# ihmcrobotics/mecano

Hardware: AMD Instinct MI355X
Metric: robot-configs/sec (RNEA+ABA), 30-DoF humanoid batch=4096 (higher is better)
Workload: dtype f64; 1 GPU; 30-DoF humanoid (SixDoF pelvis + 24 revolute), RNEA and ABA of every configuration per step, fp64, AoS [B][n] state; entry_point=mh_rnea_aba_f64, batch_per_gpu=4096, global_batch=4096, nq=31, nv=30, bodies=25, parallelism=dp1 (batch sharded, no data-path collective), kernel_variant=topo:b5c1e26c784c54fa, model_seed=43, state_seed=2342

## Files before the change

mecano_amd/csrc/mh_spec.hip:

```cpp
#include "mh_spec_kernels.h"
#include "mh_zv_kernels.h"

#include <algorithm>
#include <atomic>
#include <cstdlib>
#include <type_traits>

#ifndef MH_SPEC_PART
#define MH_SPEC_PART 0
#endif
#ifndef MH_TOPO_N
#error "MH_TOPO_N / MH_TOPO_PARENTS / MH_TOPO_TYPES must be defined"
#endif

namespace
{
struct TP
{
   static constexpr int N = MH_TOPO_N;
   static constexpr int parent[N] = {MH_TOPO_PARENTS};
   static constexpr int type[N] = {MH_TOPO_TYPES};
};
constexpr int kParents[TP::N] = {MH_TOPO_PARENTS};
constexpr int kTypes[TP::N] = {MH_TOPO_TYPES};
// ... 143 lines not shown
      return launch_lds(&mh::spec_fused_split_kernel<TP, double, ID, IO>, A, 2 * groups,
                        (size_t)split_lds_bytes(2, IO ? F_IO_LDS : 0, A.m.nq, A.m.nv), attr_bytes, stream);
   }
   else
      return hipErrorNotSupported;
}
template <int ALGO, bool ID, bool IO>
hipError_t go_split(const mh::Args<double> &A, int groups, hipStream_t stream, bool occ3 = false)
{
   if constexpr (SPL::usable())
   {
      static LdsAttr attr_bytes, attr_occ3;
      if constexpr (ALGO == 0 && ID && !IO)
      {
         if (occ3)
            return launch_lds(&mh::spec_split_kernel_occ3<TP, double, ALGO, ID, IO>, A, groups,
                              (size_t)split_lds_bytes(ALGO, 0, A.m.nq, A.m.nv), attr_occ3, stream);
      }
      return launch_lds(&mh::spec_split_kernel<TP, double, ALGO, ID, IO>, A, groups,
                        (size_t)split_lds_bytes(ALGO, IO ? F_IO_LDS : 0, A.m.nq, A.m.nv), attr_bytes, stream);
   }
   else
      return hipErrorNotSupported;
}
template <bool ID, bool IO>
hipError_t go_split_algo(int algo, const mh::Args<double> &A, int groups, hipStream_t s, bool occ3)
{
   if (algo == 2)
      return go_fused_split<ID, IO>(A, groups, s);
   if (algo == 0)
      return go_split<0, ID, IO>(A, groups, s, occ3);
   if (algo == 1)
      return go_split<1, ID, IO>(A, groups, s);
   return hipErrorNotSupported;
}

extern "C" {
#if MH_SPEC_PART != 2
int mh_spec_split_usable(void) { return SPL::usable() ? 1 : 0; }
long mh_spec_split_lds_bytes(int algo, int flags, int nq, int nv) { return split_lds_bytes(algo, flags, nq, nv); }
int mh_spec_launch_split(int algo, int flags, const void *args, int groups, void *stream)
{
   const mh::Args<double> &A = *(const mh::Args<double> *)args;
   const bool id = flags & F_IDENT, io = flags & F_IO_LDS;
   hipStream_t s = (hipStream_t)stream;
   const bool occ3 = (flags & F_OCC3) != 0;
   if (flags & F_BODIES)
   {
#ifdef MH_SPEC_MINIMAL
      return (int)hipErrorNotSupported;
#else
      if constexpr (SPL::usable())
      {
         if (id && io && (algo == 0 || algo == 1))
         {
            static LdsAttr attr0, attr1;
            const size_t lds = (size_t)split_lds_bytes(algo, F_IO_LDS, A.m.nq, A.m.nv);
            if (algo == 0)
               return (int)launch_lds(&mh::spec_split_kernel<TP, double, 0, true, true, true>, A, groups, lds, attr0, s);
            return (int)launch_lds(&mh::spec_split_kernel<TP, double, 1, true, true, true>, A, groups, lds, attr1, s);
         }
      }
      return (int)hipErrorNotSupported;
#endif
   }
   if (id && io)
      return (int)go_split_algo<true, true>(algo, A, groups, s, occ3);
#ifdef MH_SPEC_MINIMAL
   return (int)hipErrorNotSupported;
#else
   if (id)
      return (int)go_split_algo<true, false>(algo, A, groups, s, occ3);
   if (io)
      return (int)go_split_algo<false, true>(algo, A, groups, s, occ3);
   return (int)go_split_algo<false, false>(algo, A, groups, s, occ3);
#endif
}
#endif
#if MH_SPEC_PART != 1
long mh_spec_zv_lds_bytes(int nq, int nv)
{
   if constexpr (!SPL::usable())
      return 0;
   const long inertia = (long)(SPL::n_limbs() * mh::ZV_XW + SPL::ZV_TRUNK_SLOTS + nq + 2 * nv) * 64 * (long)sizeof(double);
   return std::max(inertia, split_lds_bytes(0, F_IO_LDS, nq, nv) + (long)mh::zv_bias_extra_rows<TP>() * 64 * (long)sizeof(double));
}
int mh_spec_zv_usable(void) { return SPL::usable() ? 1 : 0; }
int mh_spec_zv_self_signal(void) { return MH_ZV_TWO_STAGE && MH_ZV_SELF_SIGNAL ? 1 : 0; }
#ifdef MH_ZV_PROBE
int mh_spec_zv_probe_read(void *dst, size_t bytes) { return (int)hipMemcpyFromSymbol(dst, HIP_SYMBOL(mh::zv_probe), bytes); }
int mh_spec_zv_probe_body_read(void *dst, size_t bytes) { return (int)hipMemcpyFromSymbol(dst, HIP_SYMBOL(mh::zv_probe_body), bytes); }
#endif
int mh_spec_launch_zv(int flags, const void *args, void *taup, int *sync_flags, int *error, int epoch, int jobs, int same_l2, unsigned wait_ticks, void *stream)
{
   if constexpr (SPL::usable())
   {
      const mh::Args<double> &A = *(const mh::Args<double> *)args;
      if (!(flags & F_IO_LDS) || (jobs != 2 && jobs != 3))
         return (int)hipErrorNotSupported;
      const size_t lds = (size_t)mh_spec_zv_lds_bytes(A.m.nq, A.m.nv);
      if (lds > 160 * 1024)
         return (int)hipErrorNotSupported;
      const long groups = (A.B + 63) / 64, padded = (groups + 7) / 8 * 8;
      const mh::ZvSync sy{sync_flags, error, epoch, jobs, same_l2 ? 1 : 0, wait_ticks};
      hipStream_t s = (hipStream_t)stream;
      if (A.q_next && (!(flags & F_IDENT) || jobs != 2 || !MH_ZV_TWO_STAGE))
         return (int)hipErrorNotSupported;
      if ((flags & F_IDENT) && A.q_next)
      {
         static LdsAttr attr_step;
         auto kern = &mh::spec_zv_kernel<TP, double, true, true>;
         if (const hipError_t e = ensure_lds_attr(reinterpret_cast<const void *>(kern), lds, attr_step); e != hipSuccess)
            return (int)e;
         hipLaunchKernelGGL(kern, dim3((unsigned)(padded * jobs)), dim3(256), lds, s, A.q, A.qd, A.in3b, A.B, jobs, A, (double *)taup, sy);
         return (int)hipGetLastError();
      }
      if (flags & F_IDENT)
      {
         static LdsAttr attr;
         auto kern = &mh::spec_zv_kernel<TP, double, true>;
         if (const hipError_t e = ensure_lds_attr(reinterpret_cast<const void *>(kern), lds, attr); e != hipSuccess)
            return (int)e;
         hipLaunchKernelGGL(kern, dim3((unsigned)(padded * jobs)), dim3(256), lds, s, A.q, A.qd, A.in3b, A.B, jobs, A, (double *)taup, sy);
         return (int)hipGetLastError();
      }
#ifdef MH_SPEC_MINIMAL
      return (int)hipErrorNotSupported;
#else
      static LdsAttr attr2;
      auto kern = &mh::spec_zv_kernel<TP, double, false>;
      if (const hipError_t e = ensure_lds_attr(reinterpret_cast<const void *>(kern), lds, attr2); e != hipSuccess)
         return (int)e;
      hipLaunchKernelGGL(kern, dim3((unsigned)(padded * jobs)), dim3(256), lds, s, A.q, A.qd, A.in3b, A.B, jobs, A, (double *)taup, sy);
      return (int)hipGetLastError();
#endif
   }
   else
      return (int)hipErrorNotSupported;
}
int mh_spec_zvb_usable(void)
{
   if constexpr (SPL::usable())
      return mh::ZvbPlan<TP>::lds_slots() * 64 * (long)sizeof(double) * 2 <= 160 * 1024 ? 1 : 0;
   else
      return 0;
}
int mh_spec_zvb_cs_rows(void) { return 2 * TR::n_revolute(); }
long mh_spec_zvb_lds_bytes(int which, int nq, int nv)
{
   if constexpr (SPL::usable())
      return (long)(which == 0 ? mh::ZvbPlan<TP>::bias_lds_slots(nq, nv) : mh::ZvbPlan<TP>::lds_slots()) * 64 * (long)sizeof(double);
   else
      return 0;
}
int mh_spec_launch_zvb(int flags, const void *args, void *taup, void *cs, long cs_stride, int groups, int which, void *stream)
{
   if constexpr (SPL::usable())
   {
      const mh::Args<double> &A = *(const mh::Args<double> *)args;
      if (!(flags & F_IO_LDS) || !mh_spec_zvb_usable() || cs_stride < (A.B + 63) / 64 * 64 || groups < 1)
         return (int)hipErrorNotSupported;
      const size_t lds0 = (size_t)mh_spec_zvb_lds_bytes(0, A.m.nq, A.m.nv), lds1 = (size_t)mh_spec_zvb_lds_bytes(1, A.m.nq, A.m.nv);
      if (lds0 > 160 * 1024)
         return (int)hipErrorNotSupported;
      hipStream_t s = (hipStream_t)stream;
      auto run = [&](auto ident) -> hipError_t {
         constexpr bool ID = decltype(ident)::value;
// ... 309 lines not shown
```

mecano_amd/csrc/mh_zv_kernels.h:

```cpp
#pragma once
#include "mh_spec_kernels.h"

namespace mh
{
template <class TP>
struct ZvStore
{
   static constexpr int REG_SLOTS = Split<TP>::zv_reg_slots();
   static constexpr int kind(int j) { return Split<TP>::is_trunk(j) ? ST_LDS_KIND : ST_REG_KIND; }
   static constexpr int index(int j) { return Split<TP>::is_trunk(j) ? Split<TP>::zv_trunk_slot(j) : Split<TP>::zv_reg_slot(j); }
   static constexpr bool shared(int j) { return !Split<TP>::is_trunk(j); }
};
template <class TP>
struct ZvbStore
{
   using S = Split<TP>;
   static constexpr bool root_in_regs(int j) { return S::staged() && j == S::root(); }
   static constexpr int REG_SLOTS = S::zv_reg_slots() + (S::staged() ? Tree<TP>::zv_slots_of(S::root() < 0 ? 0 : S::root(), true) : 0);
   static constexpr int trunk_slot(int j)
   {
      int s = 0;
      for (int i = 0; i < j; i++)
         s += S::is_trunk(i) && !root_in_regs(i) ? Tree<TP>::zv_slots_of(i, false) : 0;
      return s;
// ... 427 lines not shown
         else if constexpr (MODE == 2)
            c = x_get6<Split<TP>::sub_slot(C), CX::fold_xw, 6, CX, T>(cx);
         else
            c = ZvFold<TP, C, T, CX, MODE>::run(cx);
         if constexpr (K == 0)
            pA = c;
         else
            pA = pA + c;
         children<K + 1>(cx, pA);
      }
   }
   static MH_DEV SV<T> run(const CX &cx)
   {
      MH_BODY_FENCE();
      constexpr int TYPE = TP::type[J];
      constexpr bool HAS_PARENT = TP::parent[J] >= 0;
      constexpr bool LEAF = Tree<TP>::n_children(J) == 0;
      constexpr int DO = Tree<TP>::dof_ofs(J), CO = Tree<TP>::cfg_ofs(J);
      constexpr int RS = Tree<TP>::zv_result_slot(J, CX::SPolicy::shared(J));
      const V3<T> Z{T(0), T(0), T(0)};
      SV<T> pA{Z, Z};
      if constexpr (!LEAF)
         children<0>(cx, pA);
      MH_BODY_FENCE();
      ZV_STAMP_TAIL(J, 0);
      const T *cp = cx.C + J * MC_STRIDE;
      asm volatile("" : "+s"(cp));
      const CRef<T> c{cp};
      SV<T> up{Z, Z};
      if constexpr (TYPE == JT_REVOLUTE || TYPE == JT_PRISMATIC)
      {
         T tau;
         if constexpr (CX::csmode == 3)
            tau = zvf_tau_get1<TP, J, 0, CX, T>(cx);
         else
            tau = cx.in3(DO);
         JX<T> jx;
         jx.c = T(1), jx.s = T(0), jx.d = T(0);
         if constexpr (TYPE == JT_REVOLUTE)
            jx.c = cx.st.template get<J, 7>(), jx.s = cx.st.template get<J, 8>();
         else if constexpr (HAS_PARENT)
            jx.d = cx.q(CO);
         const V3<T> sa{cx.st.template get<J, 0>(), cx.st.template get<J, 1>(), cx.st.template get<J, 2>()};
         const V3<T> sl{cx.st.template get<J, 3>(), cx.st.template get<J, 4>(), cx.st.template get<J, 5>()};
         const T dinv = cx.st.template get<J, 6>();
         const T u = tau - (TYPE == JT_REVOLUTE ? pA.a.z : pA.l.z);
         cx.st.template put<J, RS>(u * dinv);
         if constexpr (HAS_PARENT)
         {
            const XF<T> Xb = load_xb_j<TP, J, T>(c);
            const SV<T> pa = pA + SV<T>{u * sa, u * sl};
            up = force_up(TYPE, jx, Xb, pa);
         }
      }
      else if constexpr (TYPE == JT_SIXDOF)
      {
         SV<T> tau;
         if constexpr (CX::csmode == 3)
            tau = SV<T>{V3<T>{zvf_tau_get1<TP, J, 0, CX, T>(cx), zvf_tau_get1<TP, J, 1, CX, T>(cx), zvf_tau_get1<TP, J, 2, CX, T>(cx)},
                        V3<T>{zvf_tau_get1<TP, J, 3, CX, T>(cx), zvf_tau_get1<TP, J, 4, CX, T>(cx), zvf_tau_get1<TP, J, 5, CX, T>(cx)}};
         else
            tau = spec_vec<TYPE, DO, 1, CX, T>(cx, true);
         const SV<T> x = spd6_solve(st_get_ldl<J, CX, T>(cx), tau - pA);
         cx.st.template put<J, RS + 0>(x.a.x), cx.st.template put<J, RS + 1>(x.a.y), cx.st.template put<J, RS + 2>(x.a.z);
         cx.st.template put<J, RS + 3>(x.l.x), cx.st.template put<J, RS + 4>(x.l.y), cx.st.template put<J, RS + 5>(x.l.z);
         if constexpr (HAS_PARENT)
         {
            const JX<T> jx = spec_joint<TYPE, CO, CX, T>(cx);
            up = force_up(TYPE, jx, load_xb_j<TP, J, T>(c), tau);
         }
      }
      else if constexpr (HAS_PARENT)
      {
         JX<T> jx;
         jx.c = T(1), jx.s = T(0), jx.d = T(0);
         up = force_up(TYPE, jx, load_xb_j<TP, J, T>(c), pA);
      }
      MH_BODY_FENCE();
      ZV_STAMP_TAIL(J, 1);
      return up;
   }
};

template <class TP, int J, typename T, class CX, int MODE = 0>
struct ZvOut
{
   template <int K>
   static MH_DEV void children(const CX &cx, const SV<T> &a)
   {
      if constexpr (K < Tree<TP>::n_children(J))
      {
         constexpr int C = Tree<TP>::child(J, K);
         if constexpr (MODE == 1 && !Split<TP>::is_trunk(C))
         {
            if (cx.wave == Split<TP>::owner(Split<TP>::limb_index(C)))
               ZvOut<TP, C, T, CX, 0>::run(cx, a);
         }
         else
            ZvOut<TP, C, T, CX, MODE>::run(cx, a);
         children<K + 1>(cx, a);
      }
   }
   static MH_DEV void run(const CX &cx, const SV<T> &ap)
   {
      MH_BODY_FENCE();
      constexpr int TYPE = TP::type[J];
      constexpr bool HAS_PARENT = TP::parent[J] >= 0;
      constexpr bool LEAF = Tree<TP>::n_children(J) == 0;
      constexpr int DO = Tree<TP>::dof_ofs(J), CO = Tree<TP>::cfg_ofs(J);
      constexpr int RS = Tree<TP>::zv_result_slot(J, CX::SPolicy::shared(J));
      ZV_STAMP_TAIL(J, 2);
      const T *cp = cx.C + J * MC_STRIDE;
      asm volatile("" : "+s"(cp));
      const CRef<T> c{cp};
      const V3<T> Z{T(0), T(0), T(0)};
      SV<T> a{Z, Z};
      if constexpr (HAS_PARENT)
      {
         JX<T> jx;
         jx.c = T(1), jx.s = T(0), jx.d = T(0);
         if constexpr (TYPE == JT_REVOLUTE)
            jx.c = cx.st.template get<J, 7>(), jx.s = cx.st.template get<J, 8>();
         else if constexpr (TYPE != JT_FIXED)
            jx = spec_joint<TYPE, CO, CX, T>(cx);
         a = motion_down(TYPE, jx, load_xb_j<TP, J, T>(c), ap);
      }
      if constexpr (TYPE == JT_REVOLUTE || TYPE == JT_PRISMATIC)
      {
         const V3<T> sa{cx.st.template get<J, 0>(), cx.st.template get<J, 1>(), cx.st.template get<J, 2>()};
         const V3<T> sl{cx.st.template get<J, 3>(), cx.st.template get<J, 4>(), cx.st.template get<J, 5>()};
         const T qdd = cx.st.template get<J, RS>() - (dot(sa, a.a) + dot(sl, a.l));
         if (MODE == 0 || cx.wave == 0)
            cx.out(DO, qdd);
         if constexpr (TYPE == JT_REVOLUTE)
            a.a.z += qdd;
         else
            a.l.z += qdd;
      }
      else if constexpr (TYPE == JT_SIXDOF)
      {
         const SV<T> x{V3<T>{cx.st.template get<J, RS + 0>(), cx.st.template get<J, RS + 1>(), cx.st.template get<J, RS + 2>()},
                       V3<T>{cx.st.template get<J, RS + 3>(), cx.st.template get<J, RS + 4>(), cx.st.template get<J, RS + 5>()}};
         if (MODE == 0 || cx.wave == 0)
            spec_write<TYPE, DO, CX, T>(cx, x - a);
         a = x;
      }
      MH_BODY_FENCE();
      ZV_STAMP_TAIL(J, 3);
      if constexpr (!LEAF)
         children<0>(cx, a);
   }
};

template <class TP, typename T, class CX, int MODE, int K = 0>
MH_DEV void zv_roots_in(const CX &cx)
{
   if constexpr (K < Tree<TP>::n_children(-1))
   {
      (void)ZvIn<TP, Tree<TP>::child(-1, K), T, CX, MODE>::run(cx);
      zv_roots_in<TP, T, CX, MODE, K + 1>(cx);
   }
}
template <class TP, typename T, class CX, int K = 0>
MH_DEV void zv_roots_fold(const CX &cx)
{
   if constexpr (K < Tree<TP>::n_children(-1))
   {
      (void)ZvFold<TP, Tree<TP>::child(-1, K), T, CX, 1>::run(cx);
      zv_roots_fold<TP, T, CX, K + 1>(cx);
   }
}
template <class TP, typename T, class CX, int K = 0>
MH_DEV void zv_roots_out(const CX &cx)
{
   if constexpr (K < Tree<TP>::n_children(-1))
   {
      const V3<T> Z{T(0), T(0), T(0)};
      ZvOut<TP, Tree<TP>::child(-1, K), T, CX, 1>::run(cx, SV<T>{Z, Z});
      zv_roots_out<TP, T, CX, K + 1>(cx);
   }
}
template <class TP, int W, int K, int LATE, typename T, class CX>
MH_DEV void zv_limbs_in_of(const CX &cx)
{
   using S = Split<TP>;
   if constexpr (K < S::n_limbs())
   {
      if constexpr (S::owner(K) == W && (LATE < 0 || (S::is_late(K) ? 1 : 0) == LATE))
      {
         if constexpr (CX::csmode != 3 && !(CX::csmode == 0 && MH_ZV_PRE_WAVE))
            zv_pre<TP, S::limb_root(K), T, CX>(cx);
         x_put_ia<K, CX, T>(cx, ZvIn<TP, S::limb_root(K), T, CX, (LATE >= 0 && S::cut_limb(W) == K ? 3 : 0)>::run(cx));
      }
      zv_limbs_in_of<TP, W, K + 1, LATE, T, CX>(cx);
   }
}
template <class TP, int W, int I, typename T, class CX>
MH_DEV void zv_subtrunks_of(const CX &cx)
{
   using S = Split<TP>;
   if constexpr (I < S::n_sub())
   {
      constexpr int ST = S::sub_top(I);
      if constexpr (S::sub_owner(ST) == W)
         x_put_ia<S::sub_slot(ST), CX, T>(cx, ZvIn<TP, ST, T, CX, 1>::run(cx));
      zv_subtrunks_of<TP, W, I + 1, T, CX>(cx);
   }
}
template <class TP, int W, int J, typename T, class CX>
MH_DEV void zvf_park_late_tau(const CX &cx)
{
   using SP = typename CX::SPolicy;
   if constexpr (J < TP::N)
   {
      if constexpr (SP::late_body(J) && Split<TP>::owner(Split<TP>::limb_index_of_body(J)) == W)
      {
         constexpr int TS = SP::tau_slot(J), L0 = SP::late_tau_slot(J);
         cx.st.lbase[L0 * 64] = cx.st.template get<J, TS>();
         if constexpr (Tree<TP>::ndof(J) == 6)
         {
            cx.st.lbase[(L0 + 1) * 64] = cx.st.template get<J, TS + 1>(), cx.st.lbase[(L0 + 2) * 64] = cx.st.template get<J, TS + 2>();
            cx.st.lbase[(L0 + 3) * 64] = cx.st.template get<J, TS + 3>(), cx.st.lbase[(L0 + 4) * 64] = cx.st.template get<J, TS + 4>();
            cx.st.lbase[(L0 + 5) * 64] = cx.st.template get<J, TS + 5>();
         }
      }
      zvf_park_late_tau<TP, W, J + 1, T, CX>(cx);
   }
}
template <class TP, int W, typename T, class CX>
MH_DEV void zv_limbs_in(const CX &cx)
{
   using S = Split<TP>;
// ... 57 lines not shown
struct zv_relay
{
   static constexpr bool value = false;
};
template <class CX>
struct zv_relay<CX, std::enable_if_t<CX::relay>>
{
   static constexpr bool value = true;
};
template <class TP, bool RELAY = false>
struct ZvWalk
{
   using S = Split<TP>;
   static constexpr bool below(int j, int top)
   {
      for (int a = j; a >= 0; a = TP::parent[a])
         if (a == top)
            return true;
      return false;
   }
   static constexpr bool owns_late(int W)
   {
      for (int k = 0; k < S::n_limbs(); k++)
         if (S::owner(k) == W && S::is_late(k))
            return true;
      return false;
   }
   static constexpr int poster(int k)
   {
      if (!RELAY || !S::staged() || S::is_late(k) || !owns_late(S::owner(k)) || TP::parent[S::limb_root(k)] == S::root())
         return -1;
      for (int w = 0; w < 4; w++)
         if (!owns_late(w) && ZvWalk<TP, false>::needs(w, TP::parent[S::limb_root(k)]))
            return w;
      return -1;
   }
   static constexpr bool relayed(int k) { return poster(k) >= 0; }
   static constexpr bool needs(int W, int J)
   {
      for (int k = 0; k < S::n_limbs(); k++)
         if (S::owner(k) == W && below(S::limb_root(k), J) && !relayed(k))
            return true;
      return false;
   }
   static constexpr int writer(int J)
   {
      for (int w = 0; w < 4; w++)
         if (needs(w, J))
            return w;
      return 0;
   }
};
constexpr int ZV_RELAY_A = 12, ZV_RELAY_FLAG = 18;
template <class TP, int J, int W, int K, typename T, class CX>
MH_DEV void zv_relay_post(const CX &cx, const SV<T> &a)
{
   using S = Split<TP>;
   if constexpr (K < S::n_limbs())
   {
      if constexpr (TP::parent[S::limb_root(K)] == J && ZvWalk<TP, true>::poster(K) == W)
      {
         x_put6<K, ZV_XW, ZV_RELAY_A, CX, T>(cx, a);
         asm volatile("s_waitcnt lgkmcnt(0)" ::: "memory");
         __hip_atomic_store(cx.xbase + (K * ZV_XW + ZV_RELAY_FLAG) * 64, T(1), __ATOMIC_RELAXED, __HIP_MEMORY_SCOPE_WORKGROUP);
      }
      zv_relay_post<TP, J, W, K + 1, T, CX>(cx, a);
   }
}
template <class TP, int W, int K, typename T, class CX>
MH_DEV void zv_relay_clear(const CX &cx)
{
   using S = Split<TP>;
   if constexpr (K < S::n_limbs())
   {
      if constexpr (S::owner(K) == W && ZvWalk<TP, true>::relayed(K))
         x_put<K, ZV_XW, ZV_RELAY_FLAG, CX, T>(cx, T(0));
      zv_relay_clear<TP, W, K + 1, T, CX>(cx);
   }
}
template <class TP, int J, int W, typename T, class CX>
struct ZvOutW
{
   using WK = ZvWalk<TP, zv_relay<CX>::value>;
   template <int K>
   static MH_DEV void children(const CX &cx, const SV<T> &a)
   {
      if constexpr (K < Tree<TP>::n_children(J))
      {
         constexpr int C = Tree<TP>::child(J, K);
         if constexpr (!Split<TP>::is_trunk(C))
         {
            if constexpr (Split<TP>::owner(Split<TP>::limb_index(C)) == W && !WK::relayed(Split<TP>::limb_index(C)))
               ZvOut<TP, C, T, CX, 0>::run(cx, a);
         }
         else if constexpr (WK::needs(W, C))
            ZvOutW<TP, C, W, T, CX>::run(cx, a);
         children<K + 1>(cx, a);
      }
   }
   static MH_DEV void run(const CX &cx, const SV<T> &ap)
   {
      MH_BODY_FENCE();
      constexpr int TYPE = TP::type[J];
      constexpr bool HAS_PARENT = TP::parent[J] >= 0;
      constexpr int DO = Tree<TP>::dof_ofs(J), CO = Tree<TP>::cfg_ofs(J);
      constexpr int RS = Tree<TP>::zv_result_slot(J, CX::SPolicy::shared(J));
      constexpr bool WRITES = WK::writer(J) == W;
      if constexpr (WRITES)
         ZV_STAMP_TAIL(J, 2);
      const T *cp = cx.C + J * MC_STRIDE;
      asm volatile("" : "+s"(cp));
      const CRef<T> c{cp};
      const V3<T> Z{T(0), T(0), T(0)};
      SV<T> a{Z, Z};
      if constexpr (HAS_PARENT)
      {
         JX<T> jx;
         jx.c = T(1), jx.s = T(0), jx.d = T(0);
         if constexpr (TYPE == JT_REVOLUTE)
            jx.c = cx.st.template get<J, 7>(), jx.s = cx.st.template get<J, 8>();
         else if constexpr (TYPE != JT_FIXED)
            jx = spec_joint<TYPE, CO, CX, T>(cx);
         a = motion_down(TYPE, jx, load_xb_j<TP, J, T>(c), ap);
      }
      if constexpr (TYPE == JT_REVOLUTE || TYPE == JT_PRISMATIC)
      {
         const V3<T> sa{cx.st.template get<J, 0>(), cx.st.template get<J, 1>(), cx.st.template get<J, 2>()};
         const V3<T> sl{cx.st.template get<J, 3>(), cx.st.template get<J, 4>(), cx.st.template get<J, 5>()};
         const T qdd = cx.st.template get<J, RS>() - (dot(sa, a.a) + dot(sl, a.l));
         if constexpr (WRITES)
            cx.out(DO, qdd);
         if constexpr (TYPE == JT_REVOLUTE)
            a.a.z += qdd;
         else
            a.l.z += qdd;
      }
      else if constexpr (TYPE == JT_SIXDOF)
      {
         const SV<T> x{V3<T>{cx.st.template get<J, RS + 0>(), cx.st.template get<J, RS + 1>(), cx.st.template get<J, RS + 2>()},
                       V3<T>{cx.st.template get<J, RS + 3>(), cx.st.template get<J, RS + 4>(), cx.st.template get<J, RS + 5>()}};
         if constexpr (WRITES)
            spec_write<TYPE, DO, CX, T>(cx, x - a);
         a = x;
      }
      MH_BODY_FENCE();
      if constexpr (WRITES)
         ZV_STAMP_TAIL(J, 3);
      if constexpr (zv_relay<CX>::value)
         zv_relay_post<TP, J, W, 0, T, CX>(cx, a);
      children<0>(cx, a);
   }
};
template <class TP, int W, typename T, class CX, int K = 0>
MH_DEV void zv_roots_out_wave(const CX &cx)
{
   if constexpr (K < Tree<TP>::n_children(-1))
   {
      const V3<T> Z{T(0), T(0), T(0)};
      constexpr int R = Tree<TP>::child(-1, K);
      using WK = ZvWalk<TP, zv_relay<CX>::value>;
      if constexpr (WK::needs(W, R) || WK::writer(R) == W)
         ZvOutW<TP, R, W, T, CX>::run(cx, SV<T>{Z, Z});
      zv_roots_out_wave<TP, W, T, CX, K + 1>(cx);
   }
}
template <class TP, int W, int K, typename T, class CX>
MH_DEV void zv_relay_out(const CX &cx)
{
   using S = Split<TP>;
   if constexpr (K < S::n_limbs())
   {
      if constexpr (S::owner(K) == W && ZvWalk<TP, true>::relayed(K))
      {
         const lds_ptr<T> flag = cx.xbase + (K * ZV_XW + ZV_RELAY_FLAG) * 64;
         while (__builtin_amdgcn_ballot_w64(__hip_atomic_load(flag, __ATOMIC_RELAXED, __HIP_MEMORY_SCOPE_WORKGROUP) == T(0)) != 0)
            __builtin_amdgcn_s_sleep(1);
         asm volatile("" ::: "memory");
         ZvOut<TP, S::limb_root(K), T, CX, 0>::run(cx, x_get6<K, ZV_XW, ZV_RELAY_A, CX, T>(cx));
      }
      zv_relay_out<TP, W, K + 1, T, CX>(cx);
   }
}
template <class TP, int W, int K, int LATE, typename T, class CX>
MH_DEV void zv_limbs_fold_sel(const CX &cx)
{
   using S = Split<TP>;
   if constexpr (K < S::n_limbs())
   {
      if constexpr (S::owner(K) == W && (LATE < 0 || (S::is_late(K) ? 1 : 0) == LATE))
         x_put6<K, CX::fold_xw, 0, CX, T>(cx, ZvFold<TP, S::limb_root(K), T, CX, 0>::run(cx));
      zv_limbs_fold_sel<TP, W, K + 1, LATE, T, CX>(cx);
   }
}
template <class TP, int W, int I, typename T, class CX>
MH_DEV void zv_subtrunks_fold_of(const CX &cx)
{
   using S = Split<TP>;
   if constexpr (I < S::n_sub())
   {
      constexpr int ST = S::sub_top(I);
      if constexpr (S::sub_owner(ST) == W)
         x_put6<S::sub_slot(ST), CX::fold_xw, 6, CX, T>(cx, ZvFold<TP, ST, T, CX, 1>::run(cx));
      zv_subtrunks_fold_of<TP, W, I + 1, T, CX>(cx);
   }
}
struct ZvNoHook
{
   MH_DEV void after_early() const {}
   MH_DEV void after_late() const {}
   MH_DEV void before_out() const {}
};
template <class TP, int W, typename T, class CX, class HOOK = ZvNoHook>
MH_DEV void zv_fold_out(const CX &cx, const HOOK &hook = HOOK())
{
   using S = Split<TP>;
   if constexpr (W < 4)
   {
      if (cx.wave == W)
      {
         if constexpr (S::staged())
         {
#ifdef MH_ZV_PROBE
            const long k = (long)cx.own;
#endif
            if constexpr (zv_relay<CX>::value)
               zv_relay_clear<TP, W, 0, T, CX>(cx);
            zv_limbs_fold_sel<TP, W, 0, 0, T, CX>(cx);
            hook.after_early();
            ZV_STAMP(1, 7);
            zv_fold_barrier<CX>();
            zv_limbs_fold_sel<TP, W, 0, 1, T, CX>(cx);
            hook.after_late();
            zv_subtrunks_fold_of<TP, W, 0, T, CX>(cx);
            ZV_STAMP(1, 8);
            zv_fold_barrier<CX>();
            (void)ZvFold<TP, S::root(), T, CX, 2>::run(cx);
            ZV_STAMP(1, 9);
         }
         else
         {
            zv_limbs_fold_sel<TP, W, 0, -1, T, CX>(cx);
            hook.after_early();
            zv_fold_barrier<CX>();
            hook.after_late();
            zv_roots_fold<TP, T, CX>(cx);
         }
         if constexpr (CX::csmode >= 2)
            zv_fold_barrier<CX>();
         hook.before_out();
         asm volatile("" ::: "memory");
         zv_roots_out_wave<TP, W, T, CX>(cx);
         if constexpr (zv_relay<CX>::value)
            zv_relay_out<TP, W, 0, T, CX>(cx);
      }
      else
         zv_fold_out<TP, W + 1, T, CX, HOOK>(cx, hook);
   }
}

template <typename T, int N, int NT>
MH_DEV void zv_stage_rows(lds_ptr<T> dst, const T *src, int rows)
// ... 501 lines not shown
      asm volatile("" ::: "memory");
      if (active)
         zv_limbs_in<TP, 0, T, CX>(cx);
      if (rep == 0)
      {
         ZV_STAMP(1, 12);
         __syncthreads();
         ZV_STAMP(1, 13);
      }
   }
#else
   if (active)
      zv_limbs_in<TP, 0, T, CX>(cx);
#endif
   ZV_STAMP(1, 2);
   __syncthreads();
   ZV_STAMP(1, 3);
   if (active)
      zv_roots_in<TP, T, CX, (S::staged() ? 2 : 1)>(cx);
   ZV_STAMP(1, 4);
   __shared__ int zv_gave_up;
   if (wave == 0)
   {
      const bool seen = zv_wait(sy, k);
      if (lane == 0)
         zv_gave_up = seen ? 0 : 1;
   }
   __syncthreads();
   if (zv_gave_up)
   {
      for (int i = threadIdx.x; i < rows * nv; i += 256)
      {
         if constexpr (sizeof(T) == 8)
            reinterpret_cast<unsigned long long *>(A.out)[cfg0 * nv + i] = 0x7ff8000000000000ull;
         else
            reinterpret_cast<unsigned *>(A.out)[cfg0 * nv + i] = 0x7fc00000u;
      }
      return;
   }
   ZV_STAMP(1, 5);
   zv_fetch_rows<T, Tree<TP>::total_dofs(), 256>(lx, taup + cfg0 * nv, rows);
   if (threadIdx.x == 0)
   {
      __hip_atomic_store(sy.flags + k * ZV_SYNC_STRIDE, 0, __ATOMIC_RELAXED, __HIP_MEMORY_SCOPE_AGENT);
      if (sy.same_l2)
         __hip_atomic_store(sy.flags + k * ZV_SYNC_STRIDE + 32, 0, __ATOMIC_RELAXED, __HIP_MEMORY_SCOPE_AGENT);
   }
   __syncthreads();
   ZV_STAMP(1, 6);
   asm volatile("" ::: "memory");
   if (active)
      zv_fold_out<TP, 0, T, CX>(cx);
   ZV_STAMP(1, 10);
   if constexpr (!MH_ZV_DIRECT_OUT)
   {
      __syncthreads();
      wave_copy_out<T, 256>(A.out + cfg0 * nv, lres, rows * nv);
   }
   ZV_STAMP(1, 11);
}

MH_DEV bool zv_wait_word(const ZvSync &sy, const int *f)
{
   if (__hip_atomic_load(f, __ATOMIC_RELAXED, __HIP_MEMORY_SCOPE_AGENT) == sy.epoch)
      return true;
   const unsigned long long t0 = __builtin_amdgcn_s_memrealtime();
   for (;;)
   {
      __builtin_amdgcn_s_sleep(1);
      if (__hip_atomic_load(f, __ATOMIC_RELAXED, __HIP_MEMORY_SCOPE_AGENT) == sy.epoch)
         return true;
      if (__builtin_amdgcn_s_memrealtime() - t0 > (unsigned long long)sy.wait_ticks)
      {
         if ((threadIdx.x & 63) == 0)
            __hip_atomic_store(sy.error, 1, __ATOMIC_RELAXED, __HIP_MEMORY_SCOPE_SYSTEM);
         return false;
      }
   }
}
template <class TP, typename T, bool STEP>
MH_DEV void zv_aba_group2(const Args<T> &A, long k, lds_ptr<T> lds, const T *taup, const ZvSync &sy)
{
   using S = Split<TP>;
   using CX = ZvRelayCtx<Ctx<T, true, true, ZvStore<TP>, false, 0>>;
   const int wave = __builtin_amdgcn_readfirstlane((int)(threadIdx.x >> 6));
   const int lane = threadIdx.x & 63;
   constexpr int nq = Tree<TP>::total_cfgs(), nv = Tree<TP>::total_dofs();
   const lds_ptr<T> lxc = lds, lst = lxc + S::n_limbs() * ZV_XW * 64, lq = lst + S::ZV_TRUNK_SLOTS * 64, lx = lq + 64 * nq, lres = lx + 64 * nv;
   ZV_STAMP(1, 14);
   const long cfg0 = k * 64;
   const int rows = (int)(A.B - cfg0 < 64 ? A.B - cfg0 : 64);
   const bool active = lane < rows;
   __shared__ int zv_gave_up;
   if (threadIdx.x == 0)
      zv_gave_up = 0;
   ZV_STAMP(1, 0);
#if MH_ZV_SELF_SIGNAL
   const int poison = __hip_atomic_load(sy.flags + ZV_POISON_WORD, __ATOMIC_RELAXED, __HIP_MEMORY_SCOPE_AGENT);
#endif
   zv_stage_rows<T, Tree<TP>::total_cfgs(), 256>(lq, A.q + cfg0 * nq, rows);
   __syncthreads();
   ZV_STAMP(1, 1);
   CX cx;
   fill_ctx<T>(cx, A, active ? cfg0 + lane : cfg0);
   cx.lq = lq + lane * nq, cx.lqd = lq, cx.lx = lx + lane * nv, cx.lo = lres + lane * nv;
   cx.wave = wave;
   cx.xbase = lxc + lane;
   cx.st.lbase = lst + lane;
   cx.st.gbase = nullptr, cx.st.stride = 0, cx.st.lane = 0;
#ifdef MH_ZV_PROBE
   cx.own = (unsigned long long)k;
#endif
   if (active)
      zv_limbs_in<TP, 0, T, CX>(cx);
   ZV_STAMP(1, 2);
   __syncthreads();
   ZV_STAMP(1, 3);
   if (active)
      zv_roots_in<TP, T, CX, (S::staged() ? 2 : 1)>(cx);
   ZV_STAMP(1, 4);
   RowRegs<T, STEP ? Tree<TP>::total_dofs() : 1, 256> rqd;
   if constexpr (STEP)
      rqd.issue(A.qd + cfg0 * nv, rows);
   const T *const src = taup + k * 64 * nv;
   const int *const flags = sy.flags + k * ZV_SYNC_STRIDE;
   const lds_ptr<T> row = lx + lane * nv;
#if MH_ZV_SELF_SIGNAL
   bool seen;
   {
      T *const back = const_cast<T *>(src);
      if (wave == 0)
         seen = zv_take_cols<TP, T, 0>(sy, src, back, row, lane, active, poison);
      else if (wave == 1)
         seen = zv_take_cols<TP, T, 1>(sy, src, back, row, lane, active, poison);
      else if (wave == 2)
         seen = zv_take_cols<TP, T, 2>(sy, src, back, row, lane, active, poison);
      else
         seen = zv_take_cols<TP, T, 3>(sy, src, back, row, lane, active, poison);
   }
   ZV_STAMP(1, 5);
#else
   bool seen = zv_wait_word(sy, flags + 1);
   ZV_STAMP(1, 5);
   if (wave == 0)
   {
      ZvColRegs<TP, T, 0> c;
      c.issue(src, lane), c.commit(row);
   }
   else if (wave == 1)
   {
      ZvColRegs<TP, T, 1> c;
      c.issue(src, lane), c.commit(row);
   }
   else if (wave == 2)
   {
      ZvColRegs<TP, T, 2> c;
      c.issue(src, lane), c.commit(row);
   }
   else
   {
      ZvColRegs<TP, T, 3> c;
      c.issue(src, lane), c.commit(row);
   }
#endif
   const int b_first = __hip_atomic_load(flags, __ATOMIC_RELAXED, __HIP_MEMORY_SCOPE_AGENT);
   zv_lds_barrier();
   ZV_STAMP(1, 6);
   asm volatile("" ::: "memory");
   struct TrunkTau : ZvNoHook
   {
      mutable ZvColRegs<TP, T, -1> c;
      const ZvSync &sy;
      const int *flags;
      const T *src;
      lds_ptr<T> row;
      int lane, b_first;
      bool &seen;
      MH_DEV void after_early() const
      {
         if (b_first != sy.epoch)
            seen = zv_wait_word(sy, flags) && seen;
         c.issue(src, lane);
      }
      MH_DEV void after_late() const { c.commit(row); }
   };
   const TrunkTau trunk{{}, {}, sy, flags, src, row, lane, b_first, seen};
   if (active)
      zv_fold_out<TP, 0, T, CX>(cx, trunk);
   ZV_STAMP(1, 10);
   if (!seen && lane == 0)
      zv_gave_up = 1;
   __syncthreads();
   if (threadIdx.x == 0)
   {
      __hip_atomic_store(const_cast<int *>(flags), 0, __ATOMIC_RELAXED, __HIP_MEMORY_SCOPE_AGENT);
      __hip_atomic_store(const_cast<int *>(flags) + 1, 0, __ATOMIC_RELAXED, __HIP_MEMORY_SCOPE_AGENT);
   }
// ... 508 lines not shown
```

Measured before the change: 312.4 million configs/s.

## Prestage joint poses in LDS and prefetch child transforms during ABA output pass

Copies the fixed parent-to-child pose constants (rotation and offset) of every body into LDS once per workgroup. The least-loaded wave does the copy before the existing barrier. The outward ABA pass then loads each child's pose from LDS before processing the current body, which hides load latency instead of fetching scalar constants from global memory on the critical path. The cost is extra LDS space, more live registers for the per-child pose arrays, and a fill step on one wave.

```diff
diff --git a/mecano_amd/csrc/mh_spec.hip b/mecano_amd/csrc/mh_spec.hip
--- a/mecano_amd/csrc/mh_spec.hip
+++ b/mecano_amd/csrc/mh_spec.hip
@@ -249,7 +249,8 @@
 {
    if constexpr (!SPL::usable())
       return 0;
-   const long inertia = (long)(SPL::n_limbs() * mh::ZV_XW + SPL::ZV_TRUNK_SLOTS + nq + 2 * nv) * 64 * (long)sizeof(double);
+   const long inertia = (long)(SPL::n_limbs() * mh::ZV_XW + SPL::ZV_TRUNK_SLOTS + nq + 2 * nv) * 64 * (long)sizeof(double)
+                        + (long)TP::N * mh::ZV_XB_W * (long)sizeof(double);
    return std::max(inertia, split_lds_bytes(0, F_IO_LDS, nq, nv) + (long)mh::zv_bias_extra_rows<TP>() * 64 * (long)sizeof(double));
 }
 int mh_spec_zv_usable(void) { return SPL::usable() ? 1 : 0; }
diff --git a/mecano_amd/csrc/mh_zv_kernels.h b/mecano_amd/csrc/mh_zv_kernels.h
--- a/mecano_amd/csrc/mh_zv_kernels.h
+++ b/mecano_amd/csrc/mh_zv_kernels.h
@@ -533,6 +533,87 @@
    }
 };
 
+template <class TP>
+constexpr bool zv_body_below(int j, int top)
+{
+   for (int a = j; a >= 0; a = TP::parent[a])
+      if (a == top)
+         return true;
+   return false;
+}
+constexpr int ZV_XB_W = 12;
+static_assert(MC_RB == 0 && MC_PB == 9, "a pose is the first twelve constants of a joint");
+template <class CXB, typename T>
+struct ZvPrepCtx : CXB
+{
+   static constexpr bool prep = true;
+   lds_ptr<T> xpre;
+};
+template <class CX, class = void>
+struct zv_prep
+{
+   static constexpr bool value = false;
+};
+template <class CX>
+struct zv_prep<CX, std::enable_if_t<CX::prep>>
+{
+   static constexpr bool value = true;
+};
+template <class TP, int J, typename T, class CX>
+MH_DEV XF<T> zv_xb_get(const CX &cx)
+{
+   XF<T> X{};
+   if constexpr (zv_prep<CX>::value && TP::parent[J] >= 0)
+   {
+      const lds_ptr<T> p = cx.xpre + J * ZV_XB_W;
+      X.R = M3<T>{p[0], p[1], p[2], p[3], p[4], p[5], p[6], p[7], p[8]};
+      X.p = V3<T>{p[9], p[10], p[11]};
+      if constexpr (Tree<TP>::p_aligned(J))
+         X.p.y = T(0), X.p.z = T(0);
+   }
+   return X;
+}
+template <class TP>
+constexpr int zv_prep_wave()
+{
+   using S = Split<TP>;
+   int best = 3, least = 2 * TP::N + 1;
+   for (int w = 3; w >= 0; w--)
+   {
+      int n = 0;
+      for (int j = 0; j < TP::N; j++)
+         if (!S::is_trunk(j))
+            n += S::owner(S::limb_index_of_body(j)) == w ? 1 : 0;
+      if (S::staged())
+         for (int i = 0; i < S::n_sub(); i++)
+            for (int j = 0; j < TP::N; j++)
+               n += S::sub_owner(S::sub_top(i)) == w && S::is_trunk(j) && zv_body_below<TP>(j, S::sub_top(i)) ? 1 : 0;
+      if (n < least)
+         least = n, best = w;
+   }
+   return best;
+}
+template <class TP, typename T>
+MH_DEV void zv_xb_fill(lds_ptr<T> xpre, const T *C, int lane)
+{
+   constexpr int TOTAL = TP::N * ZV_XB_W, TURNS = (TOTAL + 63) / 64;
+   typedef const T __attribute__((address_space(1))) * gptr;
+   const gptr G = (gptr)(unsigned long long)C;
+   T v[TURNS];
+#pragma unroll
+   for (int i = 0; i < TURNS; i++)
+   {
+      const int e = lane + 64 * i;
+      v[i] = e < TOTAL ? G[(e / ZV_XB_W) * MC_STRIDE + e % ZV_XB_W] : T(0);
+   }
+#pragma unroll
+   for (int i = 0; i < TURNS; i++)
+   {
+      const int e = lane + 64 * i;
+      if (e < TOTAL)
+         xpre[e] = v[i];
+   }
+}
 template <class TP, int J, typename T, class CX, int MODE = 0>
 struct ZvOut
 {
@@ -552,7 +633,27 @@
          children<K + 1>(cx, a);
       }
    }
-   static MH_DEV void run(const CX &cx, const SV<T> &ap)
+   static constexpr int NC = Tree<TP>::n_children(J) > 0 ? Tree<TP>::n_children(J) : 1;
+   template <int K>
+   static MH_DEV void poses(const CX &cx, XF<T> (&xc)[NC])
+   {
+      if constexpr (K < Tree<TP>::n_children(J))
+      {
+         xc[K] = zv_xb_get<TP, Tree<TP>::child(J, K), T, CX>(cx);
+         poses<K + 1>(cx, xc);
+      }
+   }
+   template <int K>
+   static MH_DEV void children_x(const CX &cx, const SV<T> &a, const XF<T> (&xc)[NC])
+   {
+      if constexpr (K < Tree<TP>::n_children(J))
+      {
+         ZvOut<TP, Tree<TP>::child(J, K), T, CX, MODE>::go(cx, a, xc[K]);
+         children_x<K + 1>(cx, a, xc);
+      }
+   }
+   static MH_DEV void run(const CX &cx, const SV<T> &ap) { go(cx, ap, zv_xb_get<TP, J, T, CX>(cx)); }
+   static MH_DEV void go(const CX &cx, const SV<T> &ap, const XF<T> &xb)
    {
       MH_BODY_FENCE();
       constexpr int TYPE = TP::type[J];
@@ -560,6 +661,11 @@
       constexpr bool LEAF = Tree<TP>::n_children(J) == 0;
       constexpr int DO = Tree<TP>::dof_ofs(J), CO = Tree<TP>::cfg_ofs(J);
       constexpr int RS = Tree<TP>::zv_result_slot(J, CX::SPolicy::shared(J));
+      constexpr bool PREP = zv_prep<CX>::value;
+      static_assert(!PREP || MODE == 0, "a preparing context walks the trunk with ZvOutW");
+      XF<T> xc[NC];
+      if constexpr (PREP)
+         poses<0>(cx, xc);
       ZV_STAMP_TAIL(J, 2);
       const T *cp = cx.C + J * MC_STRIDE;
       asm volatile("" : "+s"(cp));
@@ -574,7 +680,10 @@
             jx.c = cx.st.template get<J, 7>(), jx.s = cx.st.template get<J, 8>();
          else if constexpr (TYPE != JT_FIXED)
             jx = spec_joint<TYPE, CO, CX, T>(cx);
-         a = motion_down(TYPE, jx, load_xb_j<TP, J, T>(c), ap);
+         if constexpr (PREP)
+            a = motion_down(TYPE, jx, xb, ap);
+         else
+            a = motion_down(TYPE, jx, load_xb_j<TP, J, T>(c), ap);
       }
       if constexpr (TYPE == JT_REVOLUTE || TYPE == JT_PRISMATIC)
       {
@@ -598,7 +707,9 @@
       }
       MH_BODY_FENCE();
       ZV_STAMP_TAIL(J, 3);
-      if constexpr (!LEAF)
+      if constexpr (!LEAF && PREP)
+         children_x<0>(cx, a, xc);
+      else if constexpr (!LEAF)
          children<0>(cx, a);
    }
 };
@@ -822,25 +933,47 @@
 struct ZvOutW
 {
    using WK = ZvWalk<TP, zv_relay<CX>::value>;
+   static constexpr int NC = Tree<TP>::n_children(J) > 0 ? Tree<TP>::n_children(J) : 1;
+   static constexpr bool walks(int C)
+   {
+      return Split<TP>::is_trunk(C) ? WK::needs(W, C) : Split<TP>::owner(Split<TP>::limb_index(C)) == W && !WK::relayed(Split<TP>::limb_index(C));
+   }
    template <int K>
-   static MH_DEV void children(const CX &cx, const SV<T> &a)
+   static MH_DEV void poses(const CX &cx, XF<T> (&xc)[NC])
+   {
+      if constexpr (K < Tree<TP>::n_children(J))
+      {
+         if constexpr (walks(Tree<TP>::child(J, K)))
+            xc[K] = zv_xb_get<TP, Tree<TP>::child(J, K), T, CX>(cx);
+         poses<K + 1>(cx, xc);
+      }
+   }
+   template <int K>
+   static MH_DEV void children(const CX &cx, const SV<T> &a, const XF<T> (&xc)[NC])
    {
       if constexpr (K < Tree<TP>::n_children(J))
       {
          constexpr int C = Tree<TP>::child(J, K);
          if constexpr (!Split<TP>::is_trunk(C))
          {
-            if constexpr (Split<TP>::owner(Split<TP>::limb_index(C)) == W && !WK::relayed(Split<TP>::limb_index(C)))
-               ZvOut<TP, C, T, CX, 0>::run(cx, a);
+            if constexpr (walks(C))
+               ZvOut<TP, C, T, CX, 0>::go(cx, a, xc[K]);
          }
-         else if constexpr (WK::needs(W, C))
-            ZvOutW<TP, C, W, T, CX>::run(cx, a);
-         children<K + 1>(cx, a);
-      }
-   }
-   static MH_DEV void run(const CX &cx, const SV<T> &ap)
+         else if constexpr (walks(C))
+            ZvOutW<TP, C, W, T, CX>::go(cx, a, xc[K]);
+         children<K + 1>(cx, a, xc);
+      }
+   }
+   static MH_DEV void run(const CX &cx, const SV<T> &ap) { go(cx, ap, zv_xb_get<TP, J, T, CX>(cx)); }
+   static MH_DEV void go(const CX &cx, const SV<T> &ap, const XF<T> &xb)
    {
       MH_BODY_FENCE();
+      constexpr bool PREP = zv_prep<CX>::value;
+      XF<T> xc[NC];
+      if constexpr (PREP)
+         poses<0>(cx, xc);
+      else
+         (void)xc;
       constexpr int TYPE = TP::type[J];
       constexpr bool HAS_PARENT = TP::parent[J] >= 0;
       constexpr int DO = Tree<TP>::dof_ofs(J), CO = Tree<TP>::cfg_ofs(J);
@@ -861,7 +994,10 @@
             jx.c = cx.st.template get<J, 7>(), jx.s = cx.st.template get<J, 8>();
          else if constexpr (TYPE != JT_FIXED)
             jx = spec_joint<TYPE, CO, CX, T>(cx);
-         a = motion_down(TYPE, jx, load_xb_j<TP, J, T>(c), ap);
+         if constexpr (PREP)
+            a = motion_down(TYPE, jx, xb, ap);
+         else
+            a = motion_down(TYPE, jx, load_xb_j<TP, J, T>(c), ap);
       }
       if constexpr (TYPE == JT_REVOLUTE || TYPE == JT_PRISMATIC)
       {
@@ -888,7 +1024,7 @@
          ZV_STAMP_TAIL(J, 3);
       if constexpr (zv_relay<CX>::value)
          zv_relay_post<TP, J, W, 0, T, CX>(cx, a);
-      children<0>(cx, a);
+      children<0>(cx, a, xc);
    }
 };
 template <class TP, int W, typename T, class CX, int K = 0>
@@ -913,10 +1049,11 @@
       if constexpr (S::owner(K) == W && ZvWalk<TP, true>::relayed(K))
       {
          const lds_ptr<T> flag = cx.xbase + (K * ZV_XW + ZV_RELAY_FLAG) * 64;
+         const XF<T> xb = zv_xb_get<TP, S::limb_root(K), T, CX>(cx);
          while (__builtin_amdgcn_ballot_w64(__hip_atomic_load(flag, __ATOMIC_RELAXED, __HIP_MEMORY_SCOPE_WORKGROUP) == T(0)) != 0)
             __builtin_amdgcn_s_sleep(1);
          asm volatile("" ::: "memory");
-         ZvOut<TP, S::limb_root(K), T, CX, 0>::run(cx, x_get6<K, ZV_XW, ZV_RELAY_A, CX, T>(cx));
+         ZvOut<TP, S::limb_root(K), T, CX, 0>::go(cx, x_get6<K, ZV_XW, ZV_RELAY_A, CX, T>(cx), xb);
       }
       zv_relay_out<TP, W, K + 1, T, CX>(cx);
    }
@@ -1584,11 +1721,12 @@
 MH_DEV void zv_aba_group2(const Args<T> &A, long k, lds_ptr<T> lds, const T *taup, const ZvSync &sy)
 {
    using S = Split<TP>;
-   using CX = ZvRelayCtx<Ctx<T, true, true, ZvStore<TP>, false, 0>>;
+   using CX = ZvPrepCtx<ZvRelayCtx<Ctx<T, true, true, ZvStore<TP>, false, 0>>, T>;
    const int wave = __builtin_amdgcn_readfirstlane((int)(threadIdx.x >> 6));
    const int lane = threadIdx.x & 63;
    constexpr int nq = Tree<TP>::total_cfgs(), nv = Tree<TP>::total_dofs();
    const lds_ptr<T> lxc = lds, lst = lxc + S::n_limbs() * ZV_XW * 64, lq = lst + S::ZV_TRUNK_SLOTS * 64, lx = lq + 64 * nq, lres = lx + 64 * nv;
+   const lds_ptr<T> lxp = lres + 64 * nv;
    ZV_STAMP(1, 14);
    const long cfg0 = k * 64;
    const int rows = (int)(A.B - cfg0 < 64 ? A.B - cfg0 : 64);
@@ -1609,12 +1747,15 @@
    cx.wave = wave;
    cx.xbase = lxc + lane;
    cx.st.lbase = lst + lane;
+   cx.xpre = lxp;
    cx.st.gbase = nullptr, cx.st.stride = 0, cx.st.lane = 0;
 #ifdef MH_ZV_PROBE
    cx.own = (unsigned long long)k;
 #endif
    if (active)
       zv_limbs_in<TP, 0, T, CX>(cx);
+   if (wave == zv_prep_wave<TP>())
+      zv_xb_fill<TP, T>(lxp, cx.C, lane);
    ZV_STAMP(1, 2);
    __syncthreads();
    ZV_STAMP(1, 3);
```

Result: slower. 261.4 million configs/s (-16.3%).
